# yongxuUSTC/DNN-for-speech-enhancement

Measured on AMD Instinct MI355X. Metric: training frames/sec (257x11 input, 3x2048 DNN), higher is better.
Workload: dtype f32; 1 GPU; C2: 2827->2048->2048->2048->257 ReLU+dropout(0.1/0.2), fp32, 256 frames/GPU/step (global bunch 256), lrate 1, momentum 0.5, 102400-frame chunk resident in HBM; parallelism=dp1, global_bunch=256, exchange=none, launcher=single process

## Files before the change

dnn-for-speech-enhancement_amd/csrc/bp_handle.h:

```cpp
#pragma once
#include <hip/hip_runtime.h>
#include <stdint.h>
#include <stdlib.h>
#include <string>
#include <vector>

#include "../../include/bp_c_api.h"

typedef uint16_t bf16_t;

extern thread_local std::string g_bp_err;
static inline int fail(int code, const std::string &msg) { g_bp_err = msg; return code; }
#define HIPCHK(x)                                                                                     \
    do {                                                                                              \
        hipError_t _e = (x);                                                                          \
        if (_e != hipSuccess)                                                                         \
            return fail(BP_ERR_DEVICE, std::string(#x) + ": " + hipGetErrorString(_e));               \
    } while (0)

static inline int pad64(int x) { return (x + 63) & ~63; }

#ifdef BP_DEV
static inline bool dev_flag(const char *name) { return getenv(name) != nullptr; }
static inline int dev_int(const char *name, int dflt) { const char *e = getenv(name); return e ? atoi(e) : dflt; }
#endif

struct StepProf;
struct bp_dp;

struct bp_handle {
    bp_config cfg;
    int L;
    int s[BP_MAXLAYER], ld[BP_MAXLAYER];
    int B, Bg;
    int cap, chunk_frames;
    hipStream_t own_stream, stream;
    float *params, *deltas;
    float *W[BP_MAXLAYER], *b[BP_MAXLAYER], *dW[BP_MAXLAYER], *db[BP_MAXLAYER];
    bp_dp *dp;
    StepProf *prof;
    const uint8_t *inj_mask[BP_MAXLAYER];
    const float *inj_x0;
    float *y[BP_MAXLAYER], *dx[BP_MAXLAYER];
    float *in, *targ, *out_dev;
    float *slabs; size_t slab_stride; int out_splits;
    unsigned *out_ticket;
    float *grad; size_t grad_floats; size_t g_off[BP_MAXLAYER], g_cnt[BP_MAXLAYER];
    float *host_out;
    float *out_chunk;
    size_t out_chunk_frames;
    uint32_t step;
    uint32_t th_vis, th_hid;
    int out_act, out_lin, out_loss;
    hipEvent_t ev0, ev1; float last_ms; int last_bunches;
    std::vector<void *> allocs;
    struct Raw { void *p; size_t bytes; };
    struct WinSet { Raw r[4]; } wset[2];
    int wcur;
    bool windows;
    struct { const float *fea, *tg, *nat; const int *ws, *tf, *nr; int D, win; } wv;
    float *x0s, *tgs;
    float *x0s2[2], *tgs2[2]; int stage_cur;
    int next_first;
    struct { bool valid; int first, tile; uint32_t step; unsigned gen; } pre;
    unsigned wgen;
    hipStream_t copy_stream;
    hipEvent_t ev_copy;
    hipEvent_t ev_retired;
    hipEvent_t ev_wretired;
    bool retired_valid, wretired_valid;
    float *in_alt, *targ_alt;
    bool bf;
    int Bp;
    bf16_t *Wb[BP_MAXLAYER];
    bf16_t *yb[BP_MAXLAYER], *ybT[BP_MAXLAYER];
    bf16_t *dxb[BP_MAXLAYER], *dxbT[BP_MAXLAYER];
    float *bf_ks_slab; unsigned *bf_ks_cnt;
    Raw wave[4], wave_pin[2];
    struct MixState *mix;
};

struct UpdateCoef { float mom, c1, wc, ndiv; };
static inline UpdateCoef update_coef(const bp_handle *h)
{
    const float m = h->cfg.momentum, lr = h->cfg.lrate;
    return {m, h->cfg.momentum_rule == 1 ? lr : (1 - m) * lr, h->cfg.weightcost, (float)h->Bg};
}

static const size_t SLACK = 4096;
int dev_alloc(bp_handle *h, float **p, size_t n_floats);

struct StepProf {
    std::vector<hipEvent_t> ev; std::vector<int> kind; size_t used;
};

hipError_t bunch(bp_handle *h, int first, bool fused);
hipError_t train_bunches(bp_handle *h, int first, int nb);
hipError_t step_inputs(bp_handle *h, int first, const float **x0, const float **tg);
hipError_t step_forward(bp_handle *h, int l, int M, const float *x0, const float *tg, float *out, bool train, float alpha);
hipError_t step_dgrad(bp_handle *h, int l);
hipError_t step_wgrads(bp_handle *h, const int *ls, int n, const float *x0, bool fused, unsigned *const *done);
bool step_wgrads_count(const bp_handle *h);
unsigned step_wgrad_tiles(const bp_handle *h, int l);
hipError_t step_shadow(bp_handle *h, int l);
bool step_stages(const bp_handle *h);
hipError_t launch_fwd(bp_handle *h, int l, int M, const float *y_prev, const float *targ, float *out, bool train, float alpha);
hipError_t launch_dgrad(bp_handle *h, int l, int M);
hipError_t launch_wgrad(bp_handle *h, int l, int M, const float *y_prev, bool fused);
hipError_t prof_mark(bp_handle *h, int kind);
int window_reserve(bp_handle *h, size_t rows_b, size_t targ_b, size_t nat_b, size_t n_samples, float **rows, float **targ, float **nat,
                   int **tables);
int window_adopt(bp_handle *h, int n_samples, int fea_dim, int context, bool nat, bool with_targ);
int out_chunk_reserve(bp_handle *h, int n_frames);
int forward_resident(bp_handle *h, int n);

void mix_free(bp_handle *h);

int dp_check(bp_handle *h);
hipError_t dp_bunch(bp_handle *h, int first);
// ... 4 lines not shown
```

dnn-for-speech-enhancement_amd/csrc/bp_step.hip:

```cpp
#include <hip/hip_runtime.h>
#include <stdio.h>
#include <stdlib.h>
#include <string.h>
#include <cmath>
#include <string>
#include <utility>
#include <vector>

#include "bp_handle.h"
#include "bp_kernels.h"
#include "bp_bf16.h"
#include "bp_wgrad_dma.h"
#include "bp_wgrad_dma_bf16.h"

thread_local std::string g_bp_err;

hipError_t prof_mark(bp_handle *h, int kind)
{
    StepProf *p = h->prof;
    if (!p) return hipSuccess;
    if (p->used == p->ev.size()) {
        hipEvent_t e; hipError_t er = hipEventCreate(&e);
        if (er != hipSuccess) return er;
        p->ev.push_back(e); p->kind.push_back(kind);
// ... 31 lines not shown
    h->allocs.push_back(q);
    *p = (float *)q;
    return BP_OK;
}

extern "C" int bp_dp_detach(bp_handle *h);
extern "C" int bp_destroy(bp_handle *h)
{
    if (!h) return BP_OK;
    (void)hipSetDevice(h->cfg.device);
    if (h->own_stream) (void)hipStreamSynchronize(h->own_stream);
    if (h->dp) (void)bp_dp_detach(h);
    for (void *p : h->allocs) (void)hipFree(p);
    for (auto &ws : h->wset) for (auto &r : ws.r) if (r.p) (void)hipFree(r.p);
    for (auto &r : h->wave) if (r.p) (void)hipFree(r.p);
    for (auto &r : h->wave_pin) if (r.p) (void)hipHostFree(r.p);
    mix_free(h);
    if (h->copy_stream) { (void)hipStreamSynchronize(h->copy_stream); (void)hipStreamDestroy(h->copy_stream); }
    if (h->ev_copy) (void)hipEventDestroy(h->ev_copy);
    if (h->ev_retired) (void)hipEventDestroy(h->ev_retired);
    if (h->ev_wretired) (void)hipEventDestroy(h->ev_wretired);
    if (h->host_out) (void)hipHostFree(h->host_out);
    if (h->out_chunk) (void)hipFree(h->out_chunk);
    if (h->ev0) (void)hipEventDestroy(h->ev0);
    if (h->ev1) (void)hipEventDestroy(h->ev1);
    if (h->own_stream) (void)hipStreamDestroy(h->own_stream);
    delete h;
    return BP_OK;
}

static int check_hyper(float, float, float, int, float, float, const char *);
static int ensure_stacked(bp_handle *h);
static int ensure_stage_tiles(bp_handle *h);
static hipError_t stage_bunch(bp_handle *h, int first, int rows, bool train);
static StageArgs stage_args(bp_handle *h, int first, int rows, bool train, int tile, uint32_t step);
static int stage_blocks(const bp_handle *h, const StageArgs &a);
static int bf_alloc(bp_handle *h, bf16_t **p, size_t n_halfs);
static hipError_t bf_shadow(bp_handle *h, int l);

enum { BF_OUT_KS = 4 };
static bool bf_out_splits(const bp_handle *h);
extern "C" int bp_create(const bp_config *cfg, const float *const *weights, const float *const *bias,
                         bp_handle **out)
{
    if (!cfg || !weights || !bias || !out) return fail(BP_ERR_ARG, "bp_create: null argument");
    if (cfg->numlayers < 2 || cfg->numlayers > BP_MAXLAYER - 1)
        return fail(BP_ERR_ARG, "bp_create: numlayers must be in 2..9");
    if (cfg->bunchsize < 1) return fail(BP_ERR_ARG, "bp_create: bunchsize must be >= 1");
    if (cfg->gpu_used < 1) return fail(BP_ERR_ARG, "bp_create: gpu_used must be >= 1");
    if (cfg->compute_dtype != 0 && cfg->compute_dtype != 1) return fail(BP_ERR_ARG, "bp_create: compute_dtype must be 0 (fp32) or 1 (bf16)");
    {
        const int r = check_hyper(cfg->lrate, cfg->momentum, cfg->weightcost, cfg->dropoutflag, cfg->visible_omit, cfg->hid_omit, "bp_create");
        if (r != BP_OK) return r;
    }
    for (int l = 0; l < cfg->numlayers; ++l)
        if (cfg->layersizes[l] < 1) return fail(BP_ERR_ARG, "bp_create: layer size must be >= 1");
    int ndev = 0;
    HIPCHK(hipGetDeviceCount(&ndev));
    if (cfg->device < 0 || cfg->device >= ndev) return fail(BP_ERR_ARG, "bp_create: device ordinal out of range");
    HIPCHK(hipSetDevice(cfg->device));

    bp_handle *h = new bp_handle();
    memset((void *)&h->cfg, 0, sizeof(h->cfg));
    h->cfg = *cfg;
    h->L = cfg->numlayers;
    h->B = cfg->bunchsize;
    h->Bg = cfg->global_bunchsize > 0 ? cfg->global_bunchsize : cfg->bunchsize;
    h->cap = cfg->max_chunk_frames > 0 ? cfg->max_chunk_frames : BP_MAXCACHEFRAME;
    if (h->cap < h->B) h->cap = h->B;
    h->chunk_frames = 0;
    h->step = 0;
    h->th_vis = cfg->dropoutflag == 1 ? drop_threshold(cfg->visible_omit) : 0u;
    h->th_hid = cfg->dropoutflag == 1 ? drop_threshold(cfg->hid_omit) : 0u;
    for (int l = 0; l < h->L; ++l) { h->s[l] = cfg->layersizes[l]; h->ld[l] = pad64(h->s[l]); }
    h->own_stream = nullptr; h->host_out = nullptr; h->ev0 = h->ev1 = nullptr;
    h->in = h->targ = h->out_dev = h->grad = nullptr; h->slabs = nullptr; h->out_splits = 1;
    h->last_ms = 0.f; h->last_bunches = 0; h->dp = nullptr; h->params = h->deltas = nullptr;
    h->next_first = -1; h->pre.valid = false; h->wgen = 0; h->stage_cur = 0;
    h->bf_ks_slab = nullptr; h->bf_ks_cnt = nullptr;
    h->out_act = h->out_lin = h->out_loss = 0;

#define CK(x) do { int _r = (x); if (_r != BP_OK) { std::string m = g_bp_err; bp_destroy(h); g_bp_err = m; return _r; } } while (0)
#define HK(x) do { hipError_t _e = (x); if (_e != hipSuccess) { std::string m = std::string(#x) + ": " + hipGetErrorString(_e); bp_destroy(h); return fail(BP_ERR_DEVICE, m); } } while (0)
    HK(hipStreamCreateWithFlags(&h->own_stream, hipStreamNonBlocking));
    h->stream = h->own_stream;
    HK(hipEventCreate(&h->ev0));
    HK(hipEventCreate(&h->ev1));
    HK(hipStreamCreateWithFlags(&h->copy_stream, hipStreamNonBlocking));
    HK(hipEventCreateWithFlags(&h->ev_copy, hipEventDisableTiming));
    HK(hipEventCreateWithFlags(&h->ev_retired, hipEventDisableTiming));
    HK(hipEventCreateWithFlags(&h->ev_wretired, hipEventDisableTiming));
    const int L = h->L;
    const size_t Bp = (size_t)((h->B + 63) & ~63);
    CK(dev_alloc(h, &h->out_dev, Bp * h->ld[L - 1]));
    if (h->ld[L - 1] <= 512 && h->ld[L - 2] >= 1024 && h->ld[L - 2] % 256 == 0) {
        h->out_splits = OUT_SPLITS;
        h->slab_stride = Bp * h->ld[L - 1];
        CK(dev_alloc(h, &h->slabs, h->slab_stride * h->out_splits));
        float *tk = nullptr;
        CK(dev_alloc(h, &tk, (Bp / 32) * (size_t)((h->ld[L - 1] + 31) / 32)));
        h->out_ticket = reinterpret_cast<unsigned *>(tk);
    }
    size_t goff = 0;
    for (int l = 1; l < L; ++l) {
        const size_t nw = (size_t)h->ld[l - 1] * h->ld[l];
        CK(dev_alloc(h, &h->y[l], Bp * h->ld[l]));
        CK(dev_alloc(h, &h->dx[l], Bp * h->ld[l]));
        h->g_off[l] = goff; h->g_cnt[l] = nw + h->ld[l]; goff += h->g_cnt[l];
    }
    h->grad_floats = goff;
    CK(dev_alloc(h, &h->params, goff));
    CK(dev_alloc(h, &h->deltas, goff));
    for (int l = 1; l < L; ++l) {
        const size_t nw = (size_t)h->ld[l - 1] * h->ld[l];
        h->W[l] = h->params + h->g_off[l]; h->b[l] = h->W[l] + nw;
        h->dW[l] = h->deltas + h->g_off[l]; h->db[l] = h->dW[l] + nw;
    }
    if (h->Bg != h->B) CK(dev_alloc(h, &h->grad, goff));
    for (int l = 1; l < L; ++l) {
        if (!weights[l] || !bias[l]) { bp_destroy(h); return fail(BP_ERR_ARG, "bp_create: weights[l]/bias[l] null"); }
        HK(hipMemcpy2DAsync(h->W[l], (size_t)h->ld[l] * 4, weights[l], (size_t)h->s[l] * 4, (size_t)h->s[l] * 4,
                            h->s[l - 1], hipMemcpyHostToDevice, h->stream));
        HK(hipMemcpyAsync(h->b[l], bias[l], (size_t)h->s[l] * 4, hipMemcpyHostToDevice, h->stream));
    }
    h->bf = cfg->compute_dtype == 1;
    h->Bp = (int)Bp;
    if (h->bf) {
        for (int l = 0; l < L; ++l) {
            const size_t act = Bp * (size_t)h->ld[l];
            if (l < L - 1) { CK(bf_alloc(h, &h->yb[l], act)); CK(bf_alloc(h, &h->ybT[l], act)); }
            if (l >= 1) {
                CK(bf_alloc(h, &h->dxb[l], act)); CK(bf_alloc(h, &h->dxbT[l], act));
                const size_t nw = (size_t)h->ld[l - 1] * h->ld[l];
                CK(bf_alloc(h, &h->Wb[l], nw));
                HK(bf_shadow(h, l));
            }
        }
        const int otiles = (int)(Bp / 32) * (h->ld[L - 1] / 64);
        if (bf_out_splits(h)) {
            CK(dev_alloc(h, &h->bf_ks_slab, (size_t)otiles * BF_OUT_KS * 128 * 16));
            float *cnt = nullptr;
            CK(dev_alloc(h, &cnt, (size_t)otiles));
            h->bf_ks_cnt = reinterpret_cast<unsigned *>(cnt);
        }
    }
    HK(hipStreamSynchronize(h->stream));
#undef CK
#undef HK
    *out = h;
    return BP_OK;
}

static int check_hyper(float lrate, float momentum, float weightcost, int dropoutflag, float visible_omit, float hid_omit, const char *who)
{
    if (!(lrate == lrate && momentum == momentum && weightcost == weightcost) || std::isinf(lrate) || std::isinf(momentum) || std::isinf(weightcost))
        return fail(BP_ERR_ARG, std::string(who) + ": lrate / momentum / weightcost must be finite");
    if (dropoutflag == 1 && !(visible_omit >= 0.0f && visible_omit < 1.0f && hid_omit >= 0.0f && hid_omit < 1.0f))
        return fail(BP_ERR_ARG, std::string(who) + ": visible_omit and hid_omit must be in [0, 1) when dropoutflag is 1");
    return BP_OK;
}

extern "C" int bp_set_hyper(bp_handle *h, float lrate, float momentum, float weightcost, int dropoutflag, float visible_omit,
                            float hid_omit)
{
    if (!h) return fail(BP_ERR_ARG, "null handle");
    int r = check_hyper(lrate, momentum, weightcost, dropoutflag, visible_omit, hid_omit, "bp_set_hyper");
// ... 81 lines not shown
        e.aux = targ; e.ldaux = cur; e.aux2 = out; e.ldaux2 = cur;
        using KOut = GemmKernel<32, 32, 64, 1, 1, true, false, EPI_OUT_SPLIT>;
        using KOutLogi = GemmKernel<32, 32, 64, 1, 1, true, false, EPI_OUT_SPLIT_LOGI>;
        const int n_gemm = g.tiles_m * g.tiles_n * OUT_SPLITS;
        StageArgs sa; memset(&sa, 0, sizeof(sa));
        int n_stage = 0;
        if (train && h->next_first >= 0) {
            const int tile = 1 - h->stage_cur;
            sa = stage_args(h, h->next_first, h->B, true, tile, h->step + 1);
            n_stage = stage_blocks(h, sa);
            h->pre.valid = true; h->pre.first = h->next_first; h->pre.tile = tile; h->pre.step = h->step + 1; h->pre.gen = h->wgen;
        }
        if (logi) hipLaunchKernelGGL(bp_out_split_stage<KOutLogi>, dim3((unsigned)(n_gemm + n_stage)), dim3(256), 0, h->stream, g, e, n_gemm, sa);
        else hipLaunchKernelGGL(bp_out_split_stage<KOut>, dim3((unsigned)(n_gemm + n_stage)), dim3(256), 0, h->stream, g, e, n_gemm, sa);
        return hipGetLastError();
    }
    e.C = train ? h->dx[l] : nullptr; e.ldc = cur;
    e.aux = targ; e.ldaux = cur; e.aux2 = out; e.ldaux2 = cur;
    if (logi) {
        if (cur <= 512) return launch<32, 32, 64, 1, 1, true, false, EPI_FWD_OUT_LOGI>(h->stream, g, e, M, cur);
        return launch<32, 64, 64, 1, 2, true, false, EPI_FWD_OUT_LOGI>(h->stream, g, e, M, cur);
    }
    if (cur <= 512) return launch<32, 32, 64, 1, 1, true, false, EPI_FWD_OUT>(h->stream, g, e, M, cur);
    return launch<32, 64, 64, 1, 2, true, false, EPI_FWD_OUT>(h->stream, g, e, M, cur);
}

enum { CFG_DGRAD_WIDE, CFG_DGRAD_WIDE128, CFG_DGRAD_NARROW, CFG_WGRAD };
struct Prepared { GemmArgs g; EpiArgs e; int M, N, cfg; bool fused; };

using KDgradWide = GemmKernel<32, 64, 64, 1, 2, true, true, EPI_DGRAD>;
using KDgradWide128 = GemmKernel<32, 64, 128, 1, 2, true, true, EPI_DGRAD>;
using KDgradNarrow = GemmKernel<32, 32, 64, 1, 1, true, true, EPI_DGRAD>;
template <int EPI> using KWgrad = GemmKernel<64, 64, 32, 2, 2, false, false, EPI>;
using KWgradStore = GemmKernel<128, 64, 16, 2, 2, false, false, EPI_WGRAD_STORE>;

static Prepared prep_dgrad(bp_handle *h, int l, int M)
{
    const int prev = h->ld[l - 1], cur = h->ld[l];
    Prepared p; memset(&p, 0, sizeof(p));
    p.g.A = h->dx[l]; p.g.lda = cur; p.g.B = h->W[l]; p.g.ldb = cur; p.g.K = cur;
    p.e = epi_zero();
    p.e.C = h->dx[l - 1]; p.e.ldc = prev; p.e.m_limit = M; p.e.n_limit = prev; p.e.n_true = h->s[l - 1];
    p.e.aux = h->y[l - 1]; p.e.ldaux = prev; p.e.act = h->cfg.activation;
    p.M = M; p.N = prev; p.cfg = prev <= 512 ? CFG_DGRAD_NARROW : (cur % 128 == 0 ? CFG_DGRAD_WIDE128 : CFG_DGRAD_WIDE);
    return p;
}

static Prepared prep_wgrad(bp_handle *h, int l, int M, const float *y_prev, bool fused)
{
    const int prev = h->ld[l - 1], cur = h->ld[l];
    Prepared p; memset(&p, 0, sizeof(p));
    p.g.A = y_prev; p.g.lda = prev; p.g.B = h->dx[l]; p.g.ldb = cur; p.g.K = M;
    p.e = epi_zero();
    p.e.ldc = cur; p.e.m_limit = prev; p.e.n_limit = cur; p.e.n_true = h->s[l];
    if (fused) {
        const UpdateCoef u = update_coef(h);
        p.e.C = h->W[l]; p.e.aux2 = h->dW[l]; p.e.ldaux2 = cur;
        p.e.mom = u.mom; p.e.c1 = u.c1; p.e.wc = u.wc; p.e.ndiv = u.ndiv;
        p.e.bias_w = h->b[l]; p.e.bias_d = h->db[l];
    } else {
        p.e.C = h->grad + h->g_off[l];
        p.e.bias_g = h->grad + h->g_off[l] + (size_t)prev * cur;
    }
    p.M = prev; p.N = cur; p.cfg = CFG_WGRAD; p.fused = fused;
    return p;
}

template <class K, int BMT, int BNT>
static hipError_t run_multi(hipStream_t st, Prepared *ps, int n)
{
    MultiArgs a; memset(&a, 0, sizeof(a));
    int t = 0;
    for (int i = 0; i < n; ++i) {
        ps[i].g.tiles_m = (ps[i].M + BMT - 1) / BMT; ps[i].g.tiles_n = (ps[i].N + BNT - 1) / BNT;
        a.g[i] = ps[i].g; a.e[i] = ps[i].e; a.first_tile[i] = t;
        t += (ps[i].g.tiles_m * ps[i].g.tiles_n + 7) & ~7;
    }
    a.first_tile[n] = t; a.n = n;
    hipLaunchKernelGGL((bp_gemm_multi<K>), dim3(t), dim3(256), 0, st, a);
    return hipGetLastError();
}

template <void (*KERNEL)(const MultiArgs)>
static hipError_t run_multi_k(hipStream_t st, Prepared *ps, int n)
{
    MultiArgs a; memset(&a, 0, sizeof(a));
    int t = 0;
    for (int i = 0; i < n; ++i) {
        ps[i].g.tiles_m = (ps[i].M + 63) / 64; ps[i].g.tiles_n = (ps[i].N + 63) / 64;
        a.g[i] = ps[i].g; a.e[i] = ps[i].e; a.first_tile[i] = t;
        t += (ps[i].g.tiles_m * ps[i].g.tiles_n + 7) & ~7;
    }
    a.first_tile[n] = t; a.n = n;
    hipLaunchKernelGGL(KERNEL, dim3(t), dim3(256), 0, st, a);
    return hipGetLastError();
}

static hipError_t run_wgrads(hipStream_t st, Prepared *ps, int n)
{
    for (int i = 0; i < n;) {
        const int m = n - i < 4 ? n - i : 4;
        int kk = ps[i].g.K;
        for (int j = 0; j < m; ++j) if (ps[i + j].g.K != kk) kk = 0;
        hipError_t er;
        if (kk == 256 && ps[i].fused) er = run_multi_k<bp_wgrad_dma<16, 4, 4, 256>>(st, ps + i, m);
        else if (kk == 128 && ps[i].fused) er = run_multi_k<bp_wgrad_dma<16, 4, 4, 128>>(st, ps + i, m);
        else if (kk == 512 && ps[i].fused) er = run_multi_k<bp_wgrad_dma<16, 4, 4, 512>>(st, ps + i, m);
        else if (kk == 256) er = run_multi_k<bp_wgrad_dma<16, 4, 4, 256, true>>(st, ps + i, m);
        else if (kk == 128) er = run_multi_k<bp_wgrad_dma<16, 4, 4, 128, true>>(st, ps + i, m);
        else if (kk == 512) er = run_multi_k<bp_wgrad_dma<16, 4, 4, 512, true>>(st, ps + i, m);
        else if (ps[i].fused) er = run_multi<KWgrad<EPI_WGRAD_UPDATE>, 64, 64>(st, ps + i, m);
        else er = run_multi<KWgradStore, 128, 64>(st, ps + i, m);
        if (er != hipSuccess) return er;
        i += m;
    }
    return hipSuccess;
}

hipError_t launch_dgrad(bp_handle *h, int l, int M)
{
    Prepared p = prep_dgrad(h, l, M);
    if (p.cfg == CFG_DGRAD_WIDE128) return run_multi<KDgradWide128, 32, 64>(h->stream, &p, 1);
    return p.cfg == CFG_DGRAD_WIDE ? run_multi<KDgradWide, 32, 64>(h->stream, &p, 1) : run_multi<KDgradNarrow, 32, 32>(h->stream, &p, 1);
}
hipError_t launch_wgrad(bp_handle *h, int l, int M, const float *y_prev, bool fused)
{
    Prepared p = prep_wgrad(h, l, M, y_prev, fused);
    return run_wgrads(h->stream, &p, 1);
}

bool step_stages(const bp_handle *h) { return h->windows || (h->th_vis != 0u && !h->inj_x0); }

static int bf_alloc(bp_handle *h, bf16_t **p, size_t n_halfs)
{
    float *q = nullptr;
    const int r = dev_alloc(h, &q, (n_halfs + 1) / 2);
    *p = (bf16_t *)q;
    return r;
}
static hipError_t bf_convert(bp_handle *h, const float *src, int lds, int rows, int cols, bf16_t *out, int ldo, bf16_t *outT,
                             int ldt, int rows_pad, int cols_pad)
{
    hipLaunchKernelGGL(bp_to_bf16_both, dim3((cols_pad + 31) / 32, (rows_pad + 31) / 32), dim3(32, 8), 0, h->stream, src, lds,
                       rows, cols, out, ldo, outT, ldt, rows_pad, cols_pad);
    return hipGetLastError();
}
static hipError_t bf_shadow(bp_handle *h, int l)
{
    const int prev = h->ld[l - 1], cur = h->ld[l];
    return bf_convert(h, h->W[l], cur, prev, cur, h->Wb[l], cur, nullptr, 0, prev, cur);
}
hipError_t step_shadow(bp_handle *h, int l) { return h->bf ? bf_shadow(h, l) : hipSuccess; }
static bool bf_out_splits(const bp_handle *h)
{
    const int L = h->L, tiles = (h->Bp / 32) * (h->ld[L - 1] / 64), nt = h->ld[L - 2] / 64;
    return h->Bp % 32 == 0 && tiles % 8 == 0 && tiles * BF_OUT_KS <= 2048 && tiles < 256 && nt >= 2 * BF_OUT_KS && nt % BF_OUT_KS == 0 && (h->Bp / 64) * (h->ld[L - 1] / 64) < 512
           && !(h->Bp % 128 == 0 && (h->Bp / 128) * (h->ld[L - 1] / 64) >= 256);
}
template <int EPI, bool BKN = false>
static hipError_t bf_launch(bp_handle *h, BfGemmArgs g, const BfEpiArgs &e, int M, int N)
{
    g.tiles_n = N / 64;
    if (M % 128 == 0 && (M / 128) * g.tiles_n >= 256) {
        g.tiles_m = M / 128;
        if constexpr (EPI == BEPI_FWD_HIDDEN || EPI == BEPI_DGRAD) {
            if ((g.tiles_n & 7) == 0 && g.lda % 8 == 0 && g.ldb % 8 == 0 && e.ldc % 8 == 0 && e.ldct % 8 == 0 && e.n_limit == N) {
                g.k_rot = EPI == BEPI_FWD_HIDDEN ? 4 : 2;
#ifdef BP_DEV
                if (EPI == BEPI_FWD_HIDDEN) g.k_rot = dev_int("BP_BF16_ROT_FWD", g.k_rot);
#endif
                hipLaunchKernelGGL((bp_gemm_bf16<EPI, 128, BKN, true>), dim3(g.tiles_m * g.tiles_n), dim3(256), 0, h->stream, g, e);
                return hipGetLastError();
            }
        }
        hipLaunchKernelGGL((bp_gemm_bf16<EPI, 128, BKN>), dim3(g.tiles_m * g.tiles_n), dim3(256), 0, h->stream, g, e);
    } else if ((M / 64) * g.tiles_n >= 512) {
        g.tiles_m = M / 64;
        hipLaunchKernelGGL((bp_gemm_bf16<EPI, 64, BKN>), dim3(g.tiles_m * g.tiles_n), dim3(256), 0, h->stream, g, e);
    } else {
        g.tiles_m = M / 32;
        if constexpr (EPI == BEPI_FWD_OUT || EPI == BEPI_FWD_OUT_LOGI) {
            if (h->bf_ks_slab && M == h->Bp && N == h->ld[h->L - 1]) {
                g.ks_slab = h->bf_ks_slab; g.ks_cnt = h->bf_ks_cnt;
                hipLaunchKernelGGL((bp_gemm_bf16<EPI, 32, BKN, false, BF_OUT_KS>), dim3(g.tiles_m * g.tiles_n * BF_OUT_KS), dim3(128), 0, h->stream, g, e);
                return hipGetLastError();
            }
        }
        hipLaunchKernelGGL((bp_gemm_bf16<EPI, 32, BKN>), dim3(g.tiles_m * g.tiles_n), dim3(128), 0, h->stream, g, e);
    }
    return hipGetLastError();
}
static hipError_t bf_fwd(bp_handle *h, int l, int M, const float *targ, float *out, bool train, float alpha)
{
    const int L = h->L, prev = h->ld[l - 1], cur = h->ld[l];
    BfGemmArgs g; memset(&g, 0, sizeof(g));
    g.A = h->yb[l - 1]; g.lda = prev; g.B = h->Wb[l]; g.ldb = cur; g.K = prev;
    BfEpiArgs e; memset(&e, 0, sizeof(e));
    e.m_limit = M; e.n_limit = cur; e.n_true = h->s[l]; e.bias = h->b[l]; e.alpha = alpha; e.act = h->cfg.activation;
    e.ldc = cur; e.ldct = h->Bp;
    if (l != L - 1) {
        e.C = h->yb[l]; e.CT = h->ybT[l];
        e.drop_thresh = train ? h->th_hid : 0u;
        e.seed_lo = (uint32_t)h->cfg.seed; e.seed_hi = (uint32_t)(h->cfg.seed >> 32);
        e.step = h->step; e.layer = (uint32_t)l; e.frame_off = h->cfg.rank_frame_offset;
        return bf_launch<BEPI_FWD_HIDDEN, true>(h, g, e, h->Bp, cur);
    }
    e.scale = 2.0f / (float)h->Bg;
    e.targ = targ; e.ldt = cur; e.out = out; e.ldo = cur;
    if (train) { e.C = h->dxb[l]; e.CT = h->dxbT[l]; }
    if (h->out_act == 1) { e.lin_cols = h->out_lin; e.loss = h->out_loss; return bf_launch<BEPI_FWD_OUT_LOGI, true>(h, g, e, h->Bp, cur); }
    return bf_launch<BEPI_FWD_OUT, true>(h, g, e, h->Bp, cur);
// ... 42 lines not shown
    for (int i0 = 0; i0 < n; i0 += BF_WGRAD_MAXP) {
        BfWgradMulti a; memset(&a, 0, sizeof(a));
        const int cnt = n - i0 < BF_WGRAD_MAXP ? n - i0 : BF_WGRAD_MAXP;
        int t = 0;
        for (int i = 0; i < cnt; ++i) {
            const int l = ls[i0 + i], prev = h->ld[l - 1], cur = h->ld[l];
            BfWgradProblem &p = a.p[i];
            p.A = h->ybT[l - 1]; p.B = h->dxbT[l]; p.ldk = h->Bp;
            p.tiles_m = prev / 64; p.tiles_n = cur / 64;
            p.e = epi_zero();
            p.e.ldc = cur; p.e.m_limit = prev; p.e.n_limit = cur; p.e.n_true = h->s[l];
            if (fused) {
                p.e.C = h->W[l]; p.e.aux2 = h->dW[l]; p.e.ldaux2 = cur;
                p.e.mom = u.mom; p.e.c1 = u.c1; p.e.wc = u.wc; p.e.ndiv = u.ndiv;
                p.e.bias_w = h->b[l]; p.e.bias_d = h->db[l];
                p.Wb = h->Wb[l]; p.ldwb = cur;
            } else {
                p.e.C = h->grad + h->g_off[l];
                p.e.bias_g = h->grad + h->g_off[l] + (size_t)prev * cur;
            }
            a.first_tile[i] = t;
            t += (p.tiles_m * p.tiles_n + 7) & ~7;
        }
        a.first_tile[cnt] = t; a.n = cnt;
#define BF_DMA_LAUNCH(K)                                                                                             \
        do { if (fused) hipLaunchKernelGGL((bp_wgrad_dma_bf16_six<K, (K >= 256 ? 64 : 32), (K >= 256 ? 3 : 4)>), dim3(t), dim3(384), 0, h->stream, a); \
             else hipLaunchKernelGGL((bp_wgrad_dma_bf16_store<K>), dim3(t), dim3(256), 0, h->stream, a); } while (0)
        switch (h->Bp) {
        case 128: BF_DMA_LAUNCH(128); break;
        case 256: BF_DMA_LAUNCH(256); break;
        case 512: BF_DMA_LAUNCH(512); break;
        default: BF_DMA_LAUNCH(1024); break;
        }
#undef BF_DMA_LAUNCH
        hipError_t er = hipGetLastError();
        if (er != hipSuccess) return er;
    }
    return hipSuccess;
}
static hipError_t bf_wgrads(bp_handle *h, const int *ls, int n, bool fused)
{
    if (bf_dma_ok(h)) return bf_wgrads_dma(h, ls, n, fused);
    for (int i = 0; i < n; ++i) { const hipError_t er = bf_wgrad(h, ls[i], fused); if (er != hipSuccess) return er; }
    return hipSuccess;
}

hipError_t step_inputs(bp_handle *h, int first, const float **x0, const float **tg)
{
    const int L = h->L, B = h->B;
    if (h->windows) {
        const hipError_t er = stage_bunch(h, first, B, true);
        *x0 = h->x0s; *tg = h->tgs;
        return er;
    }
    *x0 = h->in + (size_t)first * h->ld[0];
    *tg = h->targ + (size_t)first * h->ld[L - 1];
    if (h->inj_x0) *x0 = h->inj_x0;
    else if (step_stages(h)) {
        const hipError_t er = stage_bunch(h, first, B, true);
        *x0 = h->x0s;
        return er;
    }
    return hipSuccess;
}
hipError_t step_forward(bp_handle *h, int l, int M, const float *x0, const float *tg, float *out, bool train, float alpha)
{
    if (h->bf) {
        if (l == 1) { const hipError_t er = bf_input(h, x0, M); if (er != hipSuccess) return er; }
        return bf_fwd(h, l, M, tg, out, train, alpha);
    }
    return launch_fwd(h, l, M, l == 1 ? x0 : h->y[l - 1], tg, out, train, alpha);
}
hipError_t step_dgrad(bp_handle *h, int l) { return h->bf ? bf_dgrad(h, l) : launch_dgrad(h, l, h->B); }
bool step_wgrads_count(const bp_handle *h) { return !h->bf && (h->B == 128 || h->B == 256 || h->B == 512) && h->L - 1 <= 4; }
unsigned step_wgrad_tiles(const bp_handle *h, int l) { return (unsigned)(((h->ld[l - 1] + 63) / 64) * ((h->ld[l] + 63) / 64)); }
hipError_t step_wgrads(bp_handle *h, const int *ls, int n, const float *x0, bool fused, unsigned *const *done)
{
    if (h->bf) return bf_wgrads(h, ls, n, fused);
    Prepared ws[BP_MAXLAYER];
    for (int i = 0; i < n; ++i) {
        ws[i] = prep_wgrad(h, ls[i], h->B, ls[i] == 1 ? x0 : h->y[ls[i] - 1], fused);
        if (done) ws[i].e.done = done[ls[i]];
    }
    return run_wgrads(h->stream, ws, n);
}

hipError_t bunch(bp_handle *h, int first, bool fused)
{
    const int L = h->L;
    hipError_t er;
#define CKE(x) do { er = (x); if (er != hipSuccess) return er; } while (0)
    const float *x0, *tg;
    CKE(step_inputs(h, first, &x0, &tg));
    for (int l = 1; l < L; ++l) {
        CKE(step_forward(h, l, h->B, x0, tg, nullptr, true, 1.0f));
        CKE(prof_mark(h, l == 1 ? BP_PROF_FWD_L1 : (l == L - 1 ? BP_PROF_FWD_OUT : BP_PROF_FWD_HIDDEN)));
    }
    for (int l = L - 1; l >= 2; --l) { CKE(step_dgrad(h, l)); CKE(prof_mark(h, l == L - 1 ? BP_PROF_DGRAD_OUT : BP_PROF_DGRAD_HIDDEN)); }
    int ls[BP_MAXLAYER];
    for (int l = 1; l < L; ++l) ls[l - 1] = l;
    CKE(step_wgrads(h, ls, L - 1, x0, fused, nullptr));
    CKE(prof_mark(h, BP_PROF_WGRAD));
#undef CKE
    return hipSuccess;
}

hipError_t train_bunches(bp_handle *h, int first, int nb)
{
    hipError_t er = hipSuccess;
    for (int i = 0; i < nb && er == hipSuccess; ++i) {
        h->next_first = (step_stages(h) && !h->bf && i + 1 < nb) ? first + (i + 1) * h->B : -1;
        er = h->dp ? dp_bunch(h, first + i * h->B) : bunch(h, first + i * h->B, true);
        if (er == hipSuccess) h->step++;
    }
    h->next_first = -1; h->pre.valid = false;
    return er;
}

extern "C" int bp_upload_chunk(bp_handle *h, int n_frames, const float *in, const float *targ)
{
    if (!h || !in) return fail(BP_ERR_ARG, "bp_upload_chunk: null argument");
    if (n_frames < 0 || n_frames > h->cap) return fail(BP_ERR_ARG, "bp_upload_chunk: n_frames exceeds chunk capacity");
    HIPCHK(hipSetDevice(h->cfg.device));
    const int L = h->L;
    { const int r = ensure_stacked(h); if (r != BP_OK) return r; }
    h->windows = false;
    if (n_frames > 0) {
        if (!h->in_alt) {
            const size_t capp = (size_t)h->cap + 64;
            int r;
            if ((r = dev_alloc(h, &h->in_alt, capp * h->ld[0])) != BP_OK || (r = dev_alloc(h, &h->targ_alt, capp * h->ld[L - 1])) != BP_OK)
                return r;
            HIPCHK(hipStreamSynchronize(h->stream));
        }
        if (h->retired_valid) HIPCHK(hipStreamWaitEvent(h->copy_stream, h->ev_retired, 0));
        HIPCHK(hipMemcpy2DAsync(h->in_alt, (size_t)h->ld[0] * 4, in, (size_t)h->s[0] * 4, (size_t)h->s[0] * 4, n_frames,
                                hipMemcpyHostToDevice, h->copy_stream));
        if (targ)
            HIPCHK(hipMemcpy2DAsync(h->targ_alt, (size_t)h->ld[L - 1] * 4, targ, (size_t)h->s[L - 1] * 4,
                                    (size_t)h->s[L - 1] * 4, n_frames, hipMemcpyHostToDevice, h->copy_stream));
        HIPCHK(hipEventRecord(h->ev_copy, h->copy_stream));
        HIPCHK(hipStreamSynchronize(h->copy_stream));
        HIPCHK(hipStreamWaitEvent(h->stream, h->ev_copy, 0));
        HIPCHK(hipEventRecord(h->ev_retired, h->stream));
        h->retired_valid = true;
        std::swap(h->in, h->in_alt);
        std::swap(h->targ, h->targ_alt);
    }
    h->chunk_frames = n_frames;
    h->wgen++; h->pre.valid = false; h->next_first = -1;
    return BP_OK;
}

static int raw_reserve(bp_handle *h, int set, int which, size_t bytes)
{
    bp_handle::Raw &r = h->wset[set].r[which];
    if (bytes <= r.bytes) return BP_OK;
    if (r.p) {
        HIPCHK(hipStreamSynchronize(h->copy_stream)); HIPCHK(hipStreamSynchronize(h->stream));
        (void)hipFree(r.p); r.p = nullptr; r.bytes = 0;
    }
    const size_t want = bytes + bytes / 4 + 4096;
    hipError_t e = hipMalloc(&r.p, want);
    if (e != hipSuccess) return fail(BP_ERR_NOMEM, std::string("hipMalloc (window staging): ") + hipGetErrorString(e));
    r.bytes = want;
    return BP_OK;
}
// ... 476 lines not shown
```

dnn-for-speech-enhancement_amd/csrc/bp_wgrad_dma.h:

```cpp
#pragma once
#include "bp_kernels.h"

template <int N> struct VmWait { static __device__ __forceinline__ void go() { asm volatile("s_waitcnt vmcnt(%0)" ::"n"(N < 63 ? N : 63) : "memory"); } };

template <int BKX, int STX, int MINWG, int KTOT, bool STORE = false>
struct WgradDma {
    static constexpr int EPI = STORE ? EPI_WGRAD_STORE : EPI_WGRAD_UPDATE;
    static constexpr int NWD = STORE ? 0 : 32;
    static constexpr int BM = 64, BN = 64, BK = BKX, ST = STX, NT = KTOT / BKX, D = STX - 1;
    static constexpr int A_STAGE = BK * BM, B_STAGE = BK * BN, STAGE = A_STAGE + B_STAGE;
    static constexpr int SMEM = ST * STAGE;
    static constexpr int MIN_WG = MINWG;
    static constexpr int NA = A_STAGE / 1024, NB = B_STAGE / 1024, NDMA = NA + NB;
    static_assert(NA >= 1 && NB >= 1 && NT > D, "shape");
    typedef __attribute__((address_space(3))) void *lds_ptr;
    typedef const __attribute__((address_space(1))) void *glb_ptr;

    static __device__ __forceinline__ void issue_tile(const GemmArgs &g, int m0, int n0, int k0, float *smem, int st, int wave, int lane)
    {
#pragma unroll
        for (int i = 0; i < NA; ++i) {
            const int q = wave * NA + i, r = q * 4 + (lane >> 4), c = (lane & 15) * 4;
            __builtin_amdgcn_global_load_lds((glb_ptr)(g.A + (size_t)(k0 + r) * g.lda + m0 + c), (lds_ptr)(smem + st * STAGE + q * 256), 16, 0, 0);
        }
#pragma unroll
        for (int i = 0; i < NB; ++i) {
            const int q = wave * NB + i, r = q * 4 + (lane >> 4), c = (lane & 15) * 4;
            __builtin_amdgcn_global_load_lds((glb_ptr)(g.B + (size_t)(k0 + r) * g.ldb + n0 + c), (lds_ptr)(smem + st * STAGE + A_STAGE + q * 256), 16, 0, 0);
        }
    }
    static __device__ __forceinline__ void multiply(const float *smem, int st, int a_off, int b_off, int kh, f32x16 (&acc)[2])
    {
        constexpr int NK = BK / 2, RD = NK < 4 ? NK : 4;
        const float *ap = smem + st * STAGE + kh * BM + a_off, *bp = smem + st * STAGE + A_STAGE + kh * BN + b_off;
        float av[NK], bv[NK];
        __builtin_amdgcn_sched_barrier(0);
#pragma unroll
        for (int s = 0; s < RD; ++s) { av[s] = ap[2 * s * BM]; bv[s] = bp[2 * s * BN]; }
        __builtin_amdgcn_sched_barrier(0);
#pragma unroll
        for (int s = 0; s < NK; ++s) {
            acc[s & 1] = __builtin_amdgcn_mfma_f32_32x32x2f32(av[s], bv[s], acc[s & 1], 0, 0, 0);
            if (s + RD < NK) { av[s + RD] = ap[2 * (s + RD) * BM]; bv[s + RD] = bp[2 * (s + RD) * BN]; }
            __builtin_amdgcn_sched_barrier(0);
        }
    }
    template <int T>
    static __device__ __forceinline__ void iter(const GemmArgs &g, const EpiArgs &e, int m0, int n0, float *smem, int wave, int lane, int tid,
                                                int a_off, int b_off, int kh, int mb, int nb, bool do_bias, float &bsum, f32x16 (&acc)[2], EpiPre &pre)
    {
        if constexpr (T < NT) {
            constexpr int tiles_after = (T + D < NT ? D : NT - T) - 1;
            constexpr bool wd_out = T + D > NT;
            VmWait<tiles_after * NDMA + (wd_out ? NWD : 0)>::go();
            __builtin_amdgcn_s_barrier();
            if constexpr (T + D < NT) issue_tile(g, m0, n0, (T + D) * BK, smem, (T + D) % ST, wave, lane);
            if constexpr (T + D == NT && !STORE) epilogue_fetch<EPI_WGRAD_UPDATE, 0, 16>(e, mb, nb, lane, pre);
            if (do_bias) {
                constexpr int RPT = BK / 4;
                const float *bs = smem + (T % ST) * STAGE + A_STAGE + (tid >> 6) * RPT * BN + (tid & 63);
#pragma unroll
                for (int k = 0; k < RPT; ++k) bsum += bs[k * BN];
            }
            multiply(smem, T % ST, a_off, b_off, kh, acc);
            iter<T + 1>(g, e, m0, n0, smem, wave, lane, tid, a_off, b_off, kh, mb, nb, do_bias, bsum, acc, pre);
        }
    }
    static __device__ __forceinline__ void run(const GemmArgs &g, const EpiArgs &e, int first_block, int stride, float *smem)
    {
        const int tid = threadIdx.x, lane = tid & 63, wave = __builtin_amdgcn_readfirstlane(tid >> 6);
        const int wm = wave >> 1, wn = wave & 1;
        for (int b = first_block; b < g.tiles_m * g.tiles_n; b += stride) {
            int tile_m, tile_n;
            if ((g.tiles_n & 7) == 0) { const int xcd = b & 7, j = b >> 3, per = g.tiles_n >> 3; tile_n = xcd * per + j % per; tile_m = j / per; }
            else { tile_m = b % g.tiles_m; tile_n = b / g.tiles_m; }
            const int m0 = tile_m * BM, n0 = tile_n * BN, mb = m0 + wm * 32, nb = n0 + wn * 32;
            const int a_off = wm * 32 + (lane & 31), b_off = wn * 32 + (lane & 31), kh = lane >> 5;
            f32x16 acc[2];
#pragma unroll
            for (int r = 0; r < 16; ++r) { acc[0][r] = 0.f; acc[1][r] = 0.f; }
            const bool do_bias = tile_m == 0;
            float bsum = 0.f;
            EpiPre pre;
#pragma unroll
            for (int t = 0; t < D; ++t) issue_tile(g, m0, n0, t * BK, smem, t, wave, lane);
            iter<0>(g, e, m0, n0, smem, wave, lane, tid, a_off, b_off, kh, mb, nb, do_bias, bsum, acc, pre);
#pragma unroll
            for (int r = 0; r < 16; ++r) acc[0][r] += acc[1][r];
            __syncthreads();
            if (do_bias) {
                float *red = smem;
                red[(tid >> 6) * BN + (tid & 63)] = bsum;
                __syncthreads();
                if (tid < BN && n0 + tid < e.n_limit) {
                    const float s = (red[tid] + red[BN + tid]) + (red[2 * BN + tid] + red[3 * BN + tid]);
                    const int n = n0 + tid;
                    if constexpr (STORE) {
                        __hip_atomic_store(e.bias_g + n, s, __ATOMIC_RELAXED, __HIP_MEMORY_SCOPE_SYSTEM);
                    } else {
                        const float d = update_delta(e.mom, e.c1, 0.0f, e.ndiv, e.bias_d[n], s, e.bias_w[n]);
                        e.bias_d[n] = d;
                        e.bias_w[n] = d + 1.0f * e.bias_w[n];
                    }
                }
                __syncthreads();
            }
            epilogue_block<EPI, 0, 16>(e, mb, nb, acc[0], lane, pre);
            if constexpr (STORE) {
                if (e.done) {
                    asm volatile("s_waitcnt vmcnt(0)" ::: "memory");
                    __syncthreads();
                    if (tid == 0) __hip_atomic_fetch_add(e.done, 1u, __ATOMIC_RELAXED, __HIP_MEMORY_SCOPE_SYSTEM);
                }
            }
        }
    }
};

template <int BKX, int STX, int MINWG, int KTOT, bool STORE = false>
__global__ __launch_bounds__(256, MINWG) void bp_wgrad_dma(const MultiArgs a)
{
    using K = WgradDma<BKX, STX, MINWG, KTOT, STORE>;
    __shared__ __attribute__((aligned(16))) float smem[K::SMEM];
    const int b = blockIdx.x;
    int p = 0;
    while (p + 1 < a.n && b >= a.first_tile[p + 1]) ++p;
    K::run(a.g[p], a.e[p], b - a.first_tile[p], a.first_tile[p + 1] - a.first_tile[p], smem);
}
```

Baseline: 1.186 million frames/s.

## Make wgrad DMA kernel persistent and prefetch next tile's k-tiles across tiles

The weight-gradient kernel now launches a capped grid (default four blocks per CU, overridable by env) and each block loops over tiles across all layers in the multi-launch. While finishing one tile it issues the LDS-DMA loads for the next tile's first k-tiles into the same ring, and it splits the W/delta epilogue fetch from its use. The aim is to hide prologue load latency and cut per-block launch overhead. In exchange it needs careful vmcnt accounting and fewer barriers, which raises the risk of ordering bugs, and the grid can be smaller than the tile count.

```diff
diff --git a/dnn-for-speech-enhancement_amd/csrc/bp_handle.h b/dnn-for-speech-enhancement_amd/csrc/bp_handle.h
--- a/dnn-for-speech-enhancement_amd/csrc/bp_handle.h
+++ b/dnn-for-speech-enhancement_amd/csrc/bp_handle.h
@@ -35,6 +35,7 @@
     int B, Bg;
     int cap, chunk_frames;
     hipStream_t own_stream, stream;
+    int wgrad_slots;
     float *params, *deltas;
     float *W[BP_MAXLAYER], *b[BP_MAXLAYER], *dW[BP_MAXLAYER], *db[BP_MAXLAYER];
     bp_dp *dp;
diff --git a/dnn-for-speech-enhancement_amd/csrc/bp_step.hip b/dnn-for-speech-enhancement_amd/csrc/bp_step.hip
--- a/dnn-for-speech-enhancement_amd/csrc/bp_step.hip
+++ b/dnn-for-speech-enhancement_amd/csrc/bp_step.hip
@@ -137,6 +137,13 @@
 
 #define CK(x) do { int _r = (x); if (_r != BP_OK) { std::string m = g_bp_err; bp_destroy(h); g_bp_err = m; return _r; } } while (0)
 #define HK(x) do { hipError_t _e = (x); if (_e != hipSuccess) { std::string m = std::string(#x) + ": " + hipGetErrorString(_e); bp_destroy(h); return fail(BP_ERR_DEVICE, m); } } while (0)
+    {
+        int cus = 0;
+        HK(hipDeviceGetAttribute(&cus, hipDeviceAttributeMultiprocessorCount, cfg->device));
+        const char *ev = getenv("BP_WGRAD_SLOTS");
+        const int slots = ev ? atoi(ev) : 4 * cus;
+        h->wgrad_slots = slots < 8 ? 8 : slots & ~7;
+    }
     HK(hipStreamCreateWithFlags(&h->own_stream, hipStreamNonBlocking));
     h->stream = h->own_stream;
     HK(hipEventCreate(&h->ev0));
@@ -384,7 +391,7 @@
 }
 
 template <void (*KERNEL)(const MultiArgs)>
-static hipError_t run_multi_k(hipStream_t st, Prepared *ps, int n)
+static hipError_t run_multi_k(hipStream_t st, Prepared *ps, int n, int slots)
 {
     MultiArgs a; memset(&a, 0, sizeof(a));
     int t = 0;
@@ -394,23 +401,23 @@
         t += (ps[i].g.tiles_m * ps[i].g.tiles_n + 7) & ~7;
     }
     a.first_tile[n] = t; a.n = n;
-    hipLaunchKernelGGL(KERNEL, dim3(t), dim3(256), 0, st, a);
+    hipLaunchKernelGGL(KERNEL, dim3(t < slots ? t : slots), dim3(256), 0, st, a);
     return hipGetLastError();
 }
 
-static hipError_t run_wgrads(hipStream_t st, Prepared *ps, int n)
+static hipError_t run_wgrads(hipStream_t st, Prepared *ps, int n, int slots)
 {
     for (int i = 0; i < n;) {
         const int m = n - i < 4 ? n - i : 4;
         int kk = ps[i].g.K;
         for (int j = 0; j < m; ++j) if (ps[i + j].g.K != kk) kk = 0;
         hipError_t er;
-        if (kk == 256 && ps[i].fused) er = run_multi_k<bp_wgrad_dma<16, 4, 4, 256>>(st, ps + i, m);
-        else if (kk == 128 && ps[i].fused) er = run_multi_k<bp_wgrad_dma<16, 4, 4, 128>>(st, ps + i, m);
-        else if (kk == 512 && ps[i].fused) er = run_multi_k<bp_wgrad_dma<16, 4, 4, 512>>(st, ps + i, m);
-        else if (kk == 256) er = run_multi_k<bp_wgrad_dma<16, 4, 4, 256, true>>(st, ps + i, m);
-        else if (kk == 128) er = run_multi_k<bp_wgrad_dma<16, 4, 4, 128, true>>(st, ps + i, m);
-        else if (kk == 512) er = run_multi_k<bp_wgrad_dma<16, 4, 4, 512, true>>(st, ps + i, m);
+        if (kk == 256 && ps[i].fused) er = run_multi_k<bp_wgrad_dma<16, 4, 4, 256>>(st, ps + i, m, slots);
+        else if (kk == 128 && ps[i].fused) er = run_multi_k<bp_wgrad_dma<16, 4, 4, 128>>(st, ps + i, m, slots);
+        else if (kk == 512 && ps[i].fused) er = run_multi_k<bp_wgrad_dma<16, 4, 4, 512>>(st, ps + i, m, slots);
+        else if (kk == 256) er = run_multi_k<bp_wgrad_dma<16, 4, 4, 256, true>>(st, ps + i, m, slots);
+        else if (kk == 128) er = run_multi_k<bp_wgrad_dma<16, 4, 4, 128, true>>(st, ps + i, m, slots);
+        else if (kk == 512) er = run_multi_k<bp_wgrad_dma<16, 4, 4, 512, true>>(st, ps + i, m, slots);
         else if (ps[i].fused) er = run_multi<KWgrad<EPI_WGRAD_UPDATE>, 64, 64>(st, ps + i, m);
         else er = run_multi<KWgradStore, 128, 64>(st, ps + i, m);
         if (er != hipSuccess) return er;
@@ -428,7 +435,7 @@
 hipError_t launch_wgrad(bp_handle *h, int l, int M, const float *y_prev, bool fused)
 {
     Prepared p = prep_wgrad(h, l, M, y_prev, fused);
-    return run_wgrads(h->stream, &p, 1);
+    return run_wgrads(h->stream, &p, 1, h->wgrad_slots);
 }
 
 bool step_stages(const bp_handle *h) { return h->windows || (h->th_vis != 0u && !h->inj_x0); }
@@ -637,7 +644,7 @@
         ws[i] = prep_wgrad(h, ls[i], h->B, ls[i] == 1 ? x0 : h->y[ls[i] - 1], fused);
         if (done) ws[i].e.done = done[ls[i]];
     }
-    return run_wgrads(h->stream, ws, n);
+    return run_wgrads(h->stream, ws, n, h->wgrad_slots);
 }
 
 hipError_t bunch(bp_handle *h, int first, bool fused)
diff --git a/dnn-for-speech-enhancement_amd/csrc/bp_wgrad_dma.h b/dnn-for-speech-enhancement_amd/csrc/bp_wgrad_dma.h
--- a/dnn-for-speech-enhancement_amd/csrc/bp_wgrad_dma.h
+++ b/dnn-for-speech-enhancement_amd/csrc/bp_wgrad_dma.h
@@ -16,18 +16,74 @@
     typedef __attribute__((address_space(3))) void *lds_ptr;
     typedef const __attribute__((address_space(1))) void *glb_ptr;
 
-    static __device__ __forceinline__ void issue_tile(const GemmArgs &g, int m0, int n0, int k0, float *smem, int st, int wave, int lane)
+    static constexpr int NST = STORE ? 16 : 32;
+    static_assert(NT % ST == 0, "k-tile j of EVERY tile lies in ring stage j % ST: the ring runs on across tiles");
+    static_assert(NT >= 2 * D, "the carried head and the W/delta tail of a tile do not overlap");
+    static_assert((D - 1) * NDMA + (NWD > NST ? NWD : NST) < 64, "vmcnt is 6 bits");
+
+    struct Pos { int p, m0, n0; };
+    struct Src { const float *a, *b; int lda, ldb; };
+
+    static __device__ __forceinline__ bool decode(const MultiArgs &a, int i, Pos &t)
     {
+        int p = t.p;
+        while (p + 1 < a.n && i >= a.first_tile[p + 1]) ++p;
+        const GemmArgs &g = a.g[p];
+        const int b = i - a.first_tile[p];
+        if (b >= g.tiles_m * g.tiles_n) return false;
+        int tile_m, tile_n;
+        if ((g.tiles_n & 7) == 0) { const int xcd = b & 7, j = b >> 3, per = g.tiles_n >> 3; tile_n = xcd * per + j % per; tile_m = j / per; }
+        else { tile_m = b % g.tiles_m; tile_n = b / g.tiles_m; }
+        t.p = p; t.m0 = tile_m * BM; t.n0 = tile_n * BN;
+        return true;
+    }
+    static __device__ __forceinline__ int seek(const MultiArgs &a, int i, int stride, int total, Pos &t)
+    {
+        while (i < total && !decode(a, i, t)) i += stride;
+        return i;
+    }
+    static __device__ __forceinline__ Src src_of(const MultiArgs &a, const Pos &t)
+    {
+        const GemmArgs &g = a.g[t.p];
+        return Src{g.A + t.m0, g.B + t.n0, g.lda, g.ldb};
+    }
+
+    struct WD { float w[16], d[16]; };
+    static __device__ __forceinline__ void wd_fetch(const EpiArgs &e, int mb, int nb, int lane, WD &x)
+    {
+        const int mbc = mb < e.m_limit ? mb : 0;
+        const float *cw = uniform_ptr(e.C + (size_t)mbc * e.ldc + nb);
+        const float *cd = uniform_ptr(e.aux2 + (size_t)mbc * e.ldc + nb);
+        const unsigned ldc = __builtin_amdgcn_readfirstlane(e.ldc);
+        const unsigned lob = 4u * ((unsigned)(4 * (lane >> 5)) * (unsigned)e.ldc + (unsigned)(lane & 31));
 #pragma unroll
-        for (int i = 0; i < NA; ++i) {
-            const int q = wave * NA + i, r = q * 4 + (lane >> 4), c = (lane & 15) * 4;
-            __builtin_amdgcn_global_load_lds((glb_ptr)(g.A + (size_t)(k0 + r) * g.lda + m0 + c), (lds_ptr)(smem + st * STAGE + q * 256), 16, 0, 0);
+        for (int r = 0; r < 16; ++r) {
+            const unsigned ro = (unsigned)((r & 3) + 8 * (r >> 2)) * ldc;
+            if (r == 0) asm volatile("s_nop 4\n\tglobal_load_dword %0, %1, %2" : "=v"(x.w[r]) : "v"(lob), "s"(cw + ro) : "memory");
+            else asm volatile("global_load_dword %0, %1, %2" : "=v"(x.w[r]) : "v"(lob), "s"(cw + ro) : "memory");
+            asm volatile("global_load_dword %0, %1, %2" : "=v"(x.d[r]) : "v"(lob), "s"(cd + ro) : "memory");
+        }
+    }
+    static __device__ __forceinline__ void wd_landed(WD &x, EpiPre &pre)
+    {
+        VmWait<D * NDMA>::go();
+#pragma unroll
+        for (int r = 0; r < 16; r += 8) {
+            asm volatile("" : "+v"(x.w[r]), "+v"(x.w[r + 1]), "+v"(x.w[r + 2]), "+v"(x.w[r + 3]), "+v"(x.w[r + 4]), "+v"(x.w[r + 5]), "+v"(x.w[r + 6]), "+v"(x.w[r + 7]) :: "memory");
+            asm volatile("" : "+v"(x.d[r]), "+v"(x.d[r + 1]), "+v"(x.d[r + 2]), "+v"(x.d[r + 3]), "+v"(x.d[r + 4]), "+v"(x.d[r + 5]), "+v"(x.d[r + 6]), "+v"(x.d[r + 7]) :: "memory");
         }
 #pragma unroll
-        for (int i = 0; i < NB; ++i) {
-            const int q = wave * NB + i, r = q * 4 + (lane >> 4), c = (lane & 15) * 4;
-            __builtin_amdgcn_global_load_lds((glb_ptr)(g.B + (size_t)(k0 + r) * g.ldb + n0 + c), (lds_ptr)(smem + st * STAGE + A_STAGE + q * 256), 16, 0, 0);
-        }
+        for (int r = 0; r < 16; ++r) { pre.p0[r] = x.w[r]; pre.p1[r] = x.d[r]; }
+    }
+
+    static_assert(NA == 1 && NB == 1, "one LDS-DMA per wave, operand and k-tile");
+    static __device__ __forceinline__ unsigned lane_off(int ld, int wave, int lane) { return 4u * ((unsigned)(wave * 4 + (lane >> 4)) * (unsigned)ld + (unsigned)(lane & 15) * 4u); }
+    static __device__ __forceinline__ void issue_tile(const Src &s, int k0, float *smem, int st, int wave, int lane)
+    {
+        const char *pa = reinterpret_cast<const char *>(sgpr_row_base(s.a + (size_t)k0 * s.lda));
+        const char *pb = reinterpret_cast<const char *>(sgpr_row_base(s.b + (size_t)k0 * s.ldb));
+        __builtin_amdgcn_global_load_lds((glb_ptr)(pa + lane_off(s.lda, wave, lane)), (lds_ptr)(smem + st * STAGE + wave * 256), 16, 0, 0);
+        __builtin_amdgcn_global_load_lds((glb_ptr)(pb + lane_off(s.ldb, wave, lane)), (lds_ptr)(smem + st * STAGE + A_STAGE + wave * 256), 16, 0, 0);
     }
     static __device__ __forceinline__ void multiply(const float *smem, int st, int a_off, int b_off, int kh, f32x16 (&acc)[2])
     {
@@ -46,16 +102,17 @@
         }
     }
     template <int T>
-    static __device__ __forceinline__ void iter(const GemmArgs &g, const EpiArgs &e, int m0, int n0, float *smem, int wave, int lane, int tid,
-                                                int a_off, int b_off, int kh, int mb, int nb, bool do_bias, float &bsum, f32x16 (&acc)[2], EpiPre &pre)
+    static __device__ __forceinline__ void iter(const Src &cur, const Src &nxt, const EpiArgs &e, bool carried, float *smem, int wave, int lane, int tid,
+                                                int a_off, int b_off, int kh, int mb, int nb, bool do_bias, float &bsum, f32x16 (&acc)[2], WD &wd)
     {
         if constexpr (T < NT) {
-            constexpr int tiles_after = (T + D < NT ? D : NT - T) - 1;
-            constexpr bool wd_out = T + D > NT;
-            VmWait<tiles_after * NDMA + (wd_out ? NWD : 0)>::go();
+            constexpr int behind = (D - 1) * NDMA + (T + D > NT ? NWD : 0);
+            if constexpr (T < D) { if (carried) VmWait<behind + NST>::go(); else VmWait<behind>::go(); }
+            else VmWait<behind>::go();
             __builtin_amdgcn_s_barrier();
-            if constexpr (T + D < NT) issue_tile(g, m0, n0, (T + D) * BK, smem, (T + D) % ST, wave, lane);
-            if constexpr (T + D == NT && !STORE) epilogue_fetch<EPI_WGRAD_UPDATE, 0, 16>(e, mb, nb, lane, pre);
+            if constexpr (T + D < NT) issue_tile(cur, (T + D) * BK, smem, (T + D) % ST, wave, lane);
+            if constexpr (T + D == NT && !STORE) wd_fetch(e, mb, nb, lane, wd);
+            if constexpr (T + D >= NT) issue_tile(nxt, (T + D - NT) * BK, smem, (T + D) % ST, wave, lane);
             if (do_bias) {
                 constexpr int RPT = BK / 4;
                 const float *bs = smem + (T % ST) * STAGE + A_STAGE + (tid >> 6) * RPT * BN + (tid & 63);
@@ -63,38 +120,47 @@
                 for (int k = 0; k < RPT; ++k) bsum += bs[k * BN];
             }
             multiply(smem, T % ST, a_off, b_off, kh, acc);
-            iter<T + 1>(g, e, m0, n0, smem, wave, lane, tid, a_off, b_off, kh, mb, nb, do_bias, bsum, acc, pre);
+            iter<T + 1>(cur, nxt, e, carried, smem, wave, lane, tid, a_off, b_off, kh, mb, nb, do_bias, bsum, acc, wd);
         }
     }
-    static __device__ __forceinline__ void run(const GemmArgs &g, const EpiArgs &e, int first_block, int stride, float *smem)
+    static __device__ __forceinline__ void run(const MultiArgs &a, float *smem)
     {
         const int tid = threadIdx.x, lane = tid & 63, wave = __builtin_amdgcn_readfirstlane(tid >> 6);
         const int wm = wave >> 1, wn = wave & 1;
-        for (int b = first_block; b < g.tiles_m * g.tiles_n; b += stride) {
-            int tile_m, tile_n;
-            if ((g.tiles_n & 7) == 0) { const int xcd = b & 7, j = b >> 3, per = g.tiles_n >> 3; tile_n = xcd * per + j % per; tile_m = j / per; }
-            else { tile_m = b % g.tiles_m; tile_n = b / g.tiles_m; }
-            const int m0 = tile_m * BM, n0 = tile_n * BN, mb = m0 + wm * 32, nb = n0 + wn * 32;
+        const int stride = gridDim.x, total = a.first_tile[a.n];
+        Pos t; t.p = 0;
+        int i = seek(a, blockIdx.x, stride, total, t);
+        if (i >= total) return;
+        Src cur = src_of(a, t);
+#pragma unroll
+        for (int k = 0; k < D; ++k) issue_tile(cur, k * BK, smem, k, wave, lane);
+        bool carried = false;
+        for (;;) {
+            Pos tn = t;
+            const int in = seek(a, i + stride, stride, total, tn);
+            const bool more = in < total;
+            const Src nxt = more ? src_of(a, tn) : cur;
+            const EpiArgs &e = a.e[t.p];
+            const int mb = t.m0 + wm * 32, nb = t.n0 + wn * 32;
             const int a_off = wm * 32 + (lane & 31), b_off = wn * 32 + (lane & 31), kh = lane >> 5;
             f32x16 acc[2];
 #pragma unroll
             for (int r = 0; r < 16; ++r) { acc[0][r] = 0.f; acc[1][r] = 0.f; }
-            const bool do_bias = tile_m == 0;
+            const bool do_bias = t.m0 == 0;
             float bsum = 0.f;
-            EpiPre pre;
-#pragma unroll
-            for (int t = 0; t < D; ++t) issue_tile(g, m0, n0, t * BK, smem, t, wave, lane);
-            iter<0>(g, e, m0, n0, smem, wave, lane, tid, a_off, b_off, kh, mb, nb, do_bias, bsum, acc, pre);
+            WD wd;
+            iter<0>(cur, nxt, e, carried, smem, wave, lane, tid, a_off, b_off, kh, mb, nb, do_bias, bsum, acc, wd);
 #pragma unroll
             for (int r = 0; r < 16; ++r) acc[0][r] += acc[1][r];
-            __syncthreads();
             if (do_bias) {
-                float *red = smem;
+                float *red = smem + (ST - 1) * STAGE;
+                __builtin_amdgcn_s_barrier();
                 red[(tid >> 6) * BN + (tid & 63)] = bsum;
-                __syncthreads();
-                if (tid < BN && n0 + tid < e.n_limit) {
+                asm volatile("s_waitcnt lgkmcnt(0)" ::: "memory");
+                __builtin_amdgcn_s_barrier();
+                if (tid < BN && t.n0 + tid < e.n_limit) {
                     const float s = (red[tid] + red[BN + tid]) + (red[2 * BN + tid] + red[3 * BN + tid]);
-                    const int n = n0 + tid;
+                    const int n = t.n0 + tid;
                     if constexpr (STORE) {
                         __hip_atomic_store(e.bias_g + n, s, __ATOMIC_RELAXED, __HIP_MEMORY_SCOPE_SYSTEM);
                     } else {
@@ -103,9 +169,11 @@
                         e.bias_w[n] = d + 1.0f * e.bias_w[n];
                     }
                 }
-                __syncthreads();
             }
+            EpiPre pre;
+            if constexpr (!STORE) wd_landed(wd, pre);
             epilogue_block<EPI, 0, 16>(e, mb, nb, acc[0], lane, pre);
+            if (mb >= e.m_limit || nb >= e.n_limit) asm volatile("s_waitcnt vmcnt(0)" ::: "memory");
             if constexpr (STORE) {
                 if (e.done) {
                     asm volatile("s_waitcnt vmcnt(0)" ::: "memory");
@@ -113,7 +181,10 @@
                     if (tid == 0) __hip_atomic_fetch_add(e.done, 1u, __ATOMIC_RELAXED, __HIP_MEMORY_SCOPE_SYSTEM);
                 }
             }
+            if (!more) break;
+            t = tn; i = in; cur = nxt; carried = true;
         }
+        asm volatile("s_waitcnt vmcnt(0)" ::: "memory");
     }
 };
 
@@ -122,8 +193,5 @@
 {
     using K = WgradDma<BKX, STX, MINWG, KTOT, STORE>;
     __shared__ __attribute__((aligned(16))) float smem[K::SMEM];
-    const int b = blockIdx.x;
-    int p = 0;
-    while (p + 1 < a.n && b >= a.first_tile[p + 1]) ++p;
-    K::run(a.g[p], a.e[p], b - a.first_tile[p], a.first_tile[p + 1] - a.first_tile[p], smem);
+    K::run(a, smem);
 }
```

Measured after the change: 1.208 million frames/s, median of 6. +1.8%, better.
